# PeterChg/koordinator

Measured on AMD Instinct MI355X. Metric: pod×node Filter+Score evals/sec (LoadAwareScheduling + NodeResourcesFit, matrix mode), higher is better.
Workload: dtype int64

## Files before the change

### koordinator_amd/csrc/kg_engine.hip

```cpp
#include <dlfcn.h>
#include <hip/hip_runtime.h>
#include <rccl/rccl.h>
#include <stdarg.h>
#include <stdio.h>
#include <string.h>

#include <algorithm>
#include <map>
#include <unordered_map>
#include <utility>
#include <string>
#include <type_traits>
#include <vector>

#include "kg_comm.h"
#include "kg_common.h"
#include "kg_host.h"

#define KG_POD_CHUNK 64
#define KG_RESOLVE_THREADS 512
#define KG_RESOLVE_LA_T0 448
#define KG_CLS_ITEM_MAX 512
#define KG_MAX_CHUNK KG_PLACE_CHUNK_MAX
#define KG_MAX_TILES 4096
// ... 222 lines not shown
    if (POW2) return s >> shift;
    return (uint32_t)__builtin_fmaf((float)s, rcp, 0x1p-12f);
}

template <int S>
__device__ __forceinline__ kg_pod_hot_t<S> load_pod(const kg_pod_hot_t<S> *__restrict__ p) {
    constexpr int NB = sizeof(kg_pod_hot_t<S>) / 64;
    union U {
        kg_u32x16 v[NB];
        kg_pod_hot_t<S> h;
        __device__ U() {}
    } u;
    const kg_u32x16 *src = reinterpret_cast<const kg_u32x16 *>(p);
#pragma unroll
    for (int i = 0; i < NB; i++) u.v[i] = src[i];
    return u.h;
}

struct HotArgs {
    int32_t n_pods;
    int32_t pods_per_block;
    int32_t tile_begin;
    int32_t tiles_total;
    int64_t node_end;
    int64_t col_begin;
    int64_t score_stride;
    int32_t mask_words;
    uint32_t fit_cap;
    int32_t slot_res[8];
    int64_t now_ns;
    int32_t lax_n;
    int32_t lax_x[KG_LAX];
    uint32_t lax_w[KG_LAX];
    const double *lax_est;
};

template <int S, bool LA_PROD, bool LAX = false>
struct HotNode {
    int64_t fr[S];
    double R[S], F[S];
    double laR[2], laF0[2], laF1[2];
    double lxR[LAX ? KG_LAX : 1], lxF0[LAX ? KG_LAX : 1], lxF1[LAX ? KG_LAX : 1];
    uint32_t okbits;
    uint32_t slot_mask;
};

template <int S, bool LA_PROD, bool LAX = false>
__device__ __forceinline__ void load_hot_node(const kg_consts &c, const kg_planes &pl, const HotArgs &a, int64_t node,
                                              uint32_t slot_natives, HotNode<S, LA_PROD, LAX> &n) {
    const int64_t cap = pl.cap;
    const bool in_range = node < a.node_end;
    const uint32_t df = in_range ? pl.dflags[node] : 0u;
    const bool slow = (df & (LAX ? KGD_XSLOW : KGD_SLOW)) != 0;
    const uint32_t nfm = in_range ? pl.fit_mask[node] : 0u;
    n.slot_mask = 0;
#pragma unroll
    for (int s = 0; s < S; s++) {
        const int r = a.slot_res[s];
// ... 215 lines not shown
        __syncthreads();
        if (TOPK) {
            for (int pp = wave; pp < p1 - p0; pp += KG_BLOCK / 64) {
                const uint32_t t = tile_topk(kbuf + pp * 2 * KG_BLOCK);
                if (lane < KG_TOPK) partials[((int64_t)(p0 + pp) * a.tiles_total + tile) * KG_PARTIAL_SLOTS + lane] = t;
            }
            __syncthreads();
            continue;
        }
        const uint4 *src = reinterpret_cast<const uint4 *>(kbuf + rj * KG_BLOCK + rg * 16);
        uint32_t mx = 0;
#pragma unroll
        for (int k = 0; k < 4; k++) {
            const uint4 v = src[k];
            const uint32_t a0 = v.x > v.y ? v.x : v.y, a1 = v.z > v.w ? v.z : v.w;
            const uint32_t a2 = a0 > a1 ? a0 : a1;
            mx = mx > a2 ? mx : a2;
        }
        mx = dpp_max_step(mx, 0);
        mx = dpp_max_step(mx, 1);
        mx = dpp_max_step(mx, 2);
        mx = dpp_max_step(mx, 3);
        mx = dpp_max_step(mx, 4);
        if (rg == 31 && rj < p1 - p0) partials[(int64_t)(p0 + rj) * a.tiles_total + tile] = mx;
        __syncthreads();
    }
}

template <int NC, int NF>
struct ClsNode {
    int64_t fr[NC];
    double R[NF], F[NF];
    uint32_t w;
    uint32_t cq;
    bool ok;
    bool la_use;
};
struct ClsLa {
    double laR[2], laF[2];
};

template <int NC, int NF, bool MOST, bool FIT_ON, bool LA_ON>
__device__ __forceinline__ void load_cls_node(const kg_consts &c, const kg_planes &pl, const kg_cls_desc &d,
                                              int64_t node, int64_t node_end, int64_t now_ns, ClsNode<NC, NF> &n) {
    const int64_t cap = pl.cap;
    const bool in_range = node < node_end;
    const uint32_t df = in_range ? pl.dflags[node] : 0u;
// ... 308 lines not shown
                    __builtin_nontemporal_store(u32x4{v.x, v.y, v.z, v.w}, reinterpret_cast<u32x4 *>(scores + off + col0 + s8 * 8));
                }
            }
            if (lane < np && seg[0]) {
                uint64_t *mw = mask + (int64_t)cur[lane] * a.mask_words + (col0 >> 6);
                mw[0] = mb[0];
                if (seg[1]) mw[1] = mb[1];
            }
        }
        lds_barrier();
        if (wave == ci % (BT / 64)) {
            const int p = lane >> 3, q = lane & 7;
            const uint4 *src = reinterpret_cast<const uint4 *>(kcur + kg_kofs(p)) + q;
            uint32_t mx = 0;
#pragma unroll
            for (int k = 0; k < 16; k++) {
                const uint4 v = src[8 * k];
                mx = max(mx, max(max(v.x, v.y), max(v.z, v.w)));
            }
            mx = max(mx, (uint32_t)__builtin_amdgcn_update_dpp(0, (int)mx, 0x141, 0xf, 0xf, false));
            mx = max(mx, (uint32_t)__builtin_amdgcn_update_dpp(0, (int)mx, 0x4e, 0xf, 0xf, false));
            mx = max(mx, (uint32_t)__builtin_amdgcn_update_dpp(0, (int)mx, 0xb1, 0xf, 0xf, false));
            if (q == 0 && p < p1 - p0) {
                partials[(int64_t)cur[p] * a.tiles_total + tile] = mx;
            }
        }
    }
}

template <int NC, int NF, bool MOST, bool FIT_ON, bool LA_ON, bool OUT, bool W1>
__device__ __forceinline__ void cls_block_dup(const kg_consts &c, const kg_planes &pl, const HotArgs &a, const kg_cls_desc &d,
                                              const kg_cls_work &w, const char *__restrict__ rows_base,
                                              const int32_t *__restrict__ ids, uint64_t *__restrict__ mask,
                                              uint16_t *__restrict__ scores, uint32_t *__restrict__ partials,
                                              uint32_t *kbuf, int32_t *lid, uint16_t *lux, int32_t *cst, uint16_t *sstage,
                                              uint4 *mstage) {
    constexpr int CC = KG_EVAL3_CC;
    constexpr int BT = KG_TILE / 2;
    constexpr int SEGW = 128;
    static_assert(CC == 8 && BT == 512, "the key reduction maps one wave's lanes to 8 rows × 8 lanes");
    const int tid = threadIdx.x;
    const int lane = tid & 63;
    const int wave = __builtin_amdgcn_readfirstlane(tid >> 6);
    const int tile = a.tile_begin + w.tile;
    const int64_t wave_base = (int64_t)tile * KG_TILE + wave * SEGW;
    ClsNode<NC, NF> n[2];
    ClsLa la[2];
// ... 79 lines not shown
                        *reinterpret_cast<uint4 *>(mw) = v;
                    } else {
                        mw[0] = (uint64_t)v.x | ((uint64_t)v.y << 32);
                    }
                }
            }
        }
        if (wave == ci % (BT / 64)) {
            const int p = lane >> 3, q = lane & 7;
            const uint4 *src = reinterpret_cast<const uint4 *>(kcur + kg_kofs(p)) + q;
            uint32_t mx = 0;
#pragma unroll
            for (int k = 0; k < 16; k++) {
                const uint4 v = src[8 * k];
                mx = max(mx, max(max(v.x, v.y), max(v.z, v.w)));
            }
            mx = max(mx, (uint32_t)__builtin_amdgcn_update_dpp(0, (int)mx, 0x141, 0xf, 0xf, false));
            mx = max(mx, (uint32_t)__builtin_amdgcn_update_dpp(0, (int)mx, 0x4e, 0xf, 0xf, false));
            mx = max(mx, (uint32_t)__builtin_amdgcn_update_dpp(0, (int)mx, 0xb1, 0xf, 0xf, false));
            for (int m = m0; m < m1; m += 64) {
                const int mm = m + lane;
                const int u = mm < m1 ? lux[mm] - u0 : 0;
                const uint32_t k = (uint32_t)__builtin_amdgcn_ds_bpermute(u << 5, (int)mx);
                if (mm < m1) partials[(int64_t)lid[mm] * a.tiles_total + tile] = k;
            }
        }
    }
}

template <bool MOST, bool FIT_ON, bool LA_ON, bool OUT, bool W1, int KIND>
__global__ __launch_bounds__(KG_TILE / 2) __attribute__((amdgpu_waves_per_eu(KIND == 0 ? KG_EVAL3_WPE0 : KIND == 2 ? 5 : 4))) void k_eval3_dup(kg_consts c, kg_planes pl, HotArgs a,
                                                        const kg_cls_desc *__restrict__ descs,
                                                        const kg_cls_work *__restrict__ work, int32_t n_items,
                                                        const char *__restrict__ rows, const int32_t *__restrict__ ids,
                                                        uint64_t *__restrict__ mask, uint16_t *__restrict__ scores,
                                                        uint32_t *__restrict__ partials) {
    constexpr int CC = KG_EVAL3_CC, BT = KG_TILE / 2;
    __shared__ __attribute__((aligned(16))) uint32_t kbuf[2 * KG_KBUF_DW];
    static_assert(CC * BT <= 4096, "a chunk's keys fit the key buffer");
    __shared__ int32_t lid[KG_CLS_ITEM_MAX];
    __shared__ uint16_t lux[KG_CLS_ITEM_MAX];
    __shared__ int32_t cst[KG_CLS_ITEM_MAX / CC + 1];
    __shared__ __attribute__((aligned(16))) uint16_t sstage[OUT ? (BT / 64) * CC * 128 : 8];
    __shared__ uint4 mstage[2 * CC * 8];
    const int per = (int)(gridDim.x / KG_XCDS);
    const int item = (int)(blockIdx.x % KG_XCDS) * per + (int)(blockIdx.x / KG_XCDS);
    if (item >= n_items) return;
// ... 30 lines not shown
}

template <int VB>
__global__ __launch_bounds__(256) void k_eq_rows(const int32_t *__restrict__ of, int32_t P, const char *__restrict__ src,
                                                 char *__restrict__ dst, int64_t row_bytes) {
    typedef uint32_t vec_t __attribute__((ext_vector_type(VB / 4)));
    const int64_t nv = row_bytes / VB;
    for (int32_t p = blockIdx.y; p < P; p += gridDim.y) {
        const vec_t *s = reinterpret_cast<const vec_t *>(src + (int64_t)of[p] * row_bytes);
        vec_t *d = reinterpret_cast<vec_t *>(dst + (int64_t)p * row_bytes);
        for (int64_t i = (int64_t)blockIdx.x * blockDim.x + threadIdx.x; i < nv; i += (int64_t)gridDim.x * blockDim.x)
            __builtin_nontemporal_store(s[i], d + i);
    }
}

__global__ void k_slow_list(const uint32_t *__restrict__ dflags, int64_t begin, int64_t end, int32_t *__restrict__ list,
                            int32_t *__restrict__ count, uint32_t bit = KGD_SLOW) {
    const int64_t i = begin + (int64_t)blockIdx.x * blockDim.x + threadIdx.x;
    if (i < end && (dflags[i] & bit) && (dflags[i] & KGD_VALID)) list[atomicAdd(count, 1)] = (int32_t)i;
}

__global__ void k_fix_slow(kg_consts c, kg_planes pl, const kg_pod_dev *__restrict__ pods, int32_t n_pods,
                           const int32_t *__restrict__ list, const int32_t *__restrict__ count, int64_t col_begin,
                           int64_t col_end, int32_t mask_words, int64_t score_stride, int32_t tiles_total,
                           int64_t now_ns, unsigned long long *mask, uint16_t *scores, uint32_t *partials) {
    const int p = blockIdx.x * blockDim.x + threadIdx.x;
    if (p >= n_pods) return;
    const int32_t n = *count;
    for (int32_t k = 0; k < n; k++) {
        const int64_t node = list[k];
        if (node < col_begin || node >= col_end) continue;
        bool feas;
        uint32_t fit, la;
        kg_pair_exact(c, pl.rows[node], pl.dflags[node], pods[p], now_ns, feas, fit, la);
        const int64_t col = node - col_begin;
        if (scores) scores[(int64_t)p * score_stride + col] = (uint16_t)(fit | (la << 8));
        if (feas) {
            if (mask) atomicOr(&mask[(int64_t)p * mask_words + (col >> 6)], 1ull << (col & 63));
            const uint32_t tot = (uint32_t)c.weight_fit * fit + (uint32_t)c.weight_la * la;
            const uint32_t key = ((tot + 1u) << KG_TILE_SHIFT) | (uint32_t)(KG_TILE - 1 - (node % KG_TILE));
            atomicMax(&partials[(int64_t)p * tiles_total + node / KG_TILE], key);
        }
    }
}

__global__ __launch_bounds__(256) void k_eval_exact(kg_consts c, kg_planes pl, const kg_pod_dev *__restrict__ pods,
                                                    int32_t n_pods, int64_t begin, int64_t end, int32_t mask_words,
                                                    int64_t score_stride, int32_t tiles_total, int64_t now_ns,
                                                    unsigned long long *mask, uint16_t *scores, uint32_t *partials) {
    const int64_t col = (int64_t)blockIdx.x * 256 + threadIdx.x;
    const int64_t node = begin + col;
    const bool in = node < end;
    const uint32_t df = in ? pl.dflags[node] : 0u;
    const bool own = in && !(df & KGD_RSV);
    for (int p = blockIdx.y; p < n_pods; p += gridDim.y) {
        bool feas = false;
        uint32_t fit = 0, la = 0;
        if (own) kg_pair_exact(c, pl.rows[node], df, pods[p], now_ns, feas, fit, la);
        if (own && scores) scores[(int64_t)p * score_stride + col] = (uint16_t)(fit | (la << 8));
        const unsigned long long word = __builtin_amdgcn_ballot_w64(feas);
        if (mask && (threadIdx.x & 63) == 0 && (col >> 6) < mask_words && in) mask[(int64_t)p * mask_words + (col >> 6)] = word;
        uint32_t key = 0;
        if (feas) {
            const uint32_t tot = (uint32_t)c.weight_fit * fit + (uint32_t)c.weight_la * la;
            key = ((tot + 1u) << KG_TILE_SHIFT) | (uint32_t)(KG_TILE - 1 - (node % KG_TILE));
        }
        key = wave_max_u32(key);
        if ((threadIdx.x & 63) == 0 && key) atomicMax(&partials[(int64_t)p * tiles_total + node / KG_TILE], key);
    }
}

__global__ __launch_bounds__(256) void k_numa_bind_fix(kg_consts c, kg_planes pl, HotArgs a, const kg_pod_dev *__restrict__ pods,
                                                       unsigned long long *mask, uint16_t *scores, uint8_t *numa_scores,
                                                       uint32_t *partials) {
    const int64_t col = (int64_t)blockIdx.x * 256 + threadIdx.x;
    const int64_t node = a.col_begin + col;
    if (node >= a.node_end) return;
    const kg_node_row &row = pl.rows[node];
    if (!(row.flags & KG_NODE_NUMA_OPTIONS) || row.numa_policy == KG_NUMA_NONE || row.n_zones <= 0 ||
        !(row.flags & KG_NODE_NUMA_TOPO_VALID))
        return;
    const BatchMasks bm{0xFFu, 0xFFu};
    for (int p = blockIdx.y; p < a.n_pods; p += gridDim.y) {
        const kg_pod_dev &pd = pods[p];
        if (pd.flags & (KG_POD_NUMA_SKIP | KG_POD_NUMA_BIND_INVALID)) continue;
        const bool bind = (pd.flags & KG_POD_NUMA_CPU_BIND) ||
                          (row.node_cpu_bind != KG_NODE_CPU_BIND_NONE && pd.numa_req[KG_RES_CPU] != 0);
        if (!bind) continue;
        NodeRegs n;
        load_node(c, pl, node, true, bm, a.now_ns, n);
        uint32_t fit = 0, la = 0;
        bool ok = eval_pair(c, pl, pd, n, node, a.now_ns, fit, la);
        kg_numa_out o;
        kg_numa_pair_z<kg_zone_calc, true>(c, row, pd, o, kg_zone_calc{row});
        ok = ok && o.feasible;
        if (scores) scores[(int64_t)p * a.score_stride + col] = (uint16_t)(fit | (la << 8));
        if (numa_scores) numa_scores[(int64_t)p * a.score_stride + col] = (uint8_t)o.score;
        if (ok) {
            if (mask) atomicOr(&mask[(int64_t)p * a.mask_words + (col >> 6)], 1ull << (col & 63));
            const uint32_t key = ((total_of(c, fit, la, o.score) + 1u) << KG_TILE_SHIFT) | (uint32_t)(KG_TILE - 1 - (node % KG_TILE));
            atomicMax(&partials[(int64_t)p * a.tiles_total + node / KG_TILE], key);
        }
    }
}

#define KG_NUMA2_NODES 256
#define KG_NUMA2_SEG 32
#define KG_NUMA2_SEG_TOPK 8
#ifndef KG_NUMA2_WPE
#define KG_NUMA2_WPE 3
#endif
typedef uint32_t kg_u32x4 __attribute__((ext_vector_type(4)));
#ifndef KG_NUMA2_FLUSH
#define KG_NUMA2_FLUSH 32
#endif
#ifndef KG_NUMA2_PREFETCH
#define KG_NUMA2_PREFETCH 1
#endif
__device__ __forceinline__ void kg_glds16(const uint4 *src, uint4 *slot) {
    const uint32_t lds = __builtin_amdgcn_readfirstlane((uint32_t)(uintptr_t)slot);
    int keep;
    asm volatile("s_mov_b32 %0, m0\n\ts_mov_b32 m0, %2\n\ts_nop 0\n\tglobal_load_lds_dwordx4 %1, off\n\ts_mov_b32 m0, %0"
                 : "=&s"(keep) : "v"(src), "s"(lds) : "memory");
}
// ... 162 lines not shown
            }
            if (live && numa_scores && c0 < a.score_stride) {
                kg_u32x4 *d = reinterpret_cast<kg_u32x4 *>(numa_scores + (int64_t)p * a.score_stride + c0);
#pragma unroll
                for (int i = 0; i < FL / 16; i++)
                    __builtin_nontemporal_store(kg_u32x4{nacc[4 * i], nacc[4 * i + 1], nacc[4 * i + 2], nacc[4 * i + 3]}, d + i);
            }
#pragma unroll
            for (int i = 0; i < FL / 2; i++) sacc[i] = 0u;
#pragma unroll
            for (int i = 0; i < FL / 4; i++) nacc[i] = 0u;
        }
        if ((k & 63) == 63) {
            const int64_t c0 = col - 63;
            if (live && mask && c0 < (int64_t)a.mask_words * 64) mask[(int64_t)p * a.mask_words + (c0 >> 6)] = mword;
            mword = 0;
        }
    }
    if (npw & 63) {
        const int64_t c0 = base + npw - 32 - a.col_begin;
        if (live && mask && c0 < (int64_t)a.mask_words * 64)
            reinterpret_cast<uint32_t *>(mask + (int64_t)p * a.mask_words)[c0 >> 5] = (uint32_t)mword;
    }
    if (live && best) atomicMax(&partials[(int64_t)p * a.tiles_total + tile], best);
}

template <bool COMBINE>
__global__ __launch_bounds__(256) __attribute__((amdgpu_waves_per_eu(KG_NUMA2_WPE))) void k_eval_numa2(kg_consts c, kg_planes pl, HotArgs a,
                                                    const kg_pod_dev *__restrict__ pods,
                                                    const kg_node_row *__restrict__ rows,
                                                    unsigned long long *__restrict__ mask,
                                                    uint16_t *__restrict__ scores, uint8_t *__restrict__ numa_scores,
                                                    uint32_t *__restrict__ partials, const int32_t *__restrict__ perm,
                                                    BatchMasks bm, int32_t *queue, int32_t n_items, int32_t seg) {
    const int tid = threadIdx.x, lane = tid & 63;
    const int wave = __builtin_amdgcn_readfirstlane(tid >> 6);
    __shared__ kg_zone_tab_data ztab[256 / 64];
    __shared__ __attribute__((aligned(16))) uint4 lrow_s[256 / 64][KG_NUMA2_PREFETCH ? 2 : 1][64];
    static_assert(sizeof(kg_node_row) % 16 == 0 && sizeof(kg_node_row) <= 64 * 16, "rows are staged as 16-byte words");
    const int n_pb = (a.n_pods + 63) / 64;
    for (int it = 0;; it++) {
        int64_t tile, base;
        int npw, pb;
        if (queue == nullptr) {
            if (it > 0) break;
            tile = (int64_t)a.tile_begin + blockIdx.x;
            pb = blockIdx.y;
// ... 5 lines not shown
            item = __builtin_amdgcn_readfirstlane(item);
            if (item >= n_items) break;
            pb = item % n_pb;
            const int run = item / n_pb;
            tile = (int64_t)a.tile_begin + run / (KG_TILE / seg);
            base = (int64_t)a.tile_begin * KG_TILE + (int64_t)run * seg;
            npw = seg;
        }
        const int slot = pb * 64 + lane;
        const bool live = slot < a.n_pods;
        const int p = live && perm ? perm[slot] : slot;
        const kg_pod_dev pd = pods[live ? p : 0];
        numa2_run<COMBINE>(c, pl, a, pd, p, live, tile, base, npw, rows, mask, scores, numa_scores, partials, bm, ztab[wave],
                  &lrow_s[wave][0][0]);
    }
}

__device__ __forceinline__ unsigned long long decode_partial(uint32_t k, int tile) {
    if (k == 0) return 0ull;
    const uint32_t node = (uint32_t)tile * KG_TILE + (KG_TILE - 1) - (k & (KG_TILE - 1));
    return ((unsigned long long)(k >> KG_TILE_SHIFT) << 32) | (0xFFFFFFFFull - node);
}

__global__ void k_top1(const uint32_t *__restrict__ partials, int32_t tiles, int32_t n_pods,
                       unsigned long long *__restrict__ out) {
    const int wave = (blockIdx.x * blockDim.x + threadIdx.x) >> 6;
    const int lane = threadIdx.x & 63;
    if (wave >= n_pods) return;
    unsigned long long best = 0;
    for (int t = lane; t < tiles; t += 64) {
        unsigned long long k = decode_partial(partials[(int64_t)wave * tiles + t], t);
        best = best > k ? best : k;
    }
    best = wave_max_u64(best);
    if (lane == 0) out[wave] = best;
}

template <bool NUMA>
__device__ unsigned long long pair_key(const kg_consts &c, const kg_planes &pl, const kg_pod_dev &p, int64_t node,
                                       int64_t n_nodes, int64_t now_ns) {
    if (node < 0 || node >= n_nodes) return 0ull;
    NodeRegs n;
    BatchMasks bm{0xFFu, 0xFFu};
    load_node(c, pl, node, true, bm, now_ns, n);
    uint32_t fit, la, numa = 0;
    if (!eval_pair(c, pl, p, n, node, now_ns, fit, la)) return 0ull;
    if (NUMA && (c.plugins & KG_PLUGIN_NUMA)) {
        const uint64_t ns = kg_numa_eval_any(c, pl.rows[node], p);
        if (!(ns >> 32)) return 0ull;
        numa = (uint32_t)ns;
    }
    return ((unsigned long long)(total_of(c, fit, la, numa) + 1u) << 32) | (0xFFFFFFFFull - (unsigned long long)node);
}

#define KG_NUMA_CHUNK_PODS 16
#define KG_CHUNK_WPE 3
template <bool BZ>
__global__ __launch_bounds__(256) __attribute__((amdgpu_waves_per_eu(KG_CHUNK_WPE))) void k_eval_numa_chunk(kg_consts c, kg_planes pl, HotArgs a,
// ... 1693 lines not shown
            hipLaunchKernelGGL((k_eval3_dup<MOST, FIT_ON, LA_ON, true, W1, KIND>), g1, dim3(KG_TILE / 2), 0, stream,
                               e->consts, e->pl, a, descs, work + first, count, rows, ids, mask, scores, partials);
        else
            hipLaunchKernelGGL((k_eval3_dup<MOST, FIT_ON, LA_ON, false, W1, KIND>), g1, dim3(KG_TILE / 2), 0, stream,
                               e->consts, e->pl, a, descs, work + first, count, rows, ids, mask, scores, partials);
    } else {
        grid.y = (unsigned)count;
        if (mask)
            hipLaunchKernelGGL((k_eval3<MOST, FIT_ON, LA_ON, true, W1, KIND, LAU>), grid, dim3(KG_TILE / 2), 0, stream,
                               e->consts, e->pl, a, descs, work + first, rows, ids, mask, scores, partials);
        else
            hipLaunchKernelGGL((k_eval3<MOST, FIT_ON, LA_ON, false, W1, KIND, LAU>), grid, dim3(KG_TILE / 2), 0, stream,
                               e->consts, e->pl, a, descs, work + first, rows, ids, mask, scores, partials);
    }
}

template <bool MOST, bool FIT_ON, bool LA_ON, bool W1>
void launch_cls4(kg_engine *e, dim3 grid, const HotArgs &a, uint64_t *mask, uint16_t *scores, uint32_t *partials) {
    const char *m = (const char *)e->cls_mem;
    const kg_cls_desc *descs = (const kg_cls_desc *)m;
    const kg_cls_work *work = (const kg_cls_work *)(m + e->cls_work_off);
    const char *rows = m + e->cls_rows_off;
    const int32_t *ids = (const int32_t *)(m + e->cls_ids_off);
    if (!e->stream2) {
        (void)hipStreamCreateWithFlags(&e->stream2, hipStreamNonBlocking);
        (void)hipEventCreateWithFlags(&e->ev_fork, hipEventDisableTiming);
        (void)hipEventCreateWithFlags(&e->ev_join, hipEventDisableTiming);
    }
    (void)hipEventRecord(e->ev_fork, e->stream);
    (void)hipStreamWaitEvent(e->stream2, e->ev_fork, 0);
    hipStream_t s2 = e->stream2;
#define KG_LAUNCH_KIND(K)                                                                                              \
    launch_cls_kind<MOST, FIT_ON, LA_ON, W1, K, 2>(e, grid, a, descs, work, rows, ids, mask, scores, partials, e->stream); \
    launch_cls_kind<MOST, FIT_ON, LA_ON, W1, K, 1>(e, grid, a, descs, work, rows, ids, mask, scores, partials, e->stream); \
    launch_cls_kind<MOST, FIT_ON, LA_ON, W1, K, 0>(e, grid, a, descs, work, rows, ids, mask, scores, partials, s2)
    KG_LAUNCH_KIND(0);
    KG_LAUNCH_KIND(1);
    KG_LAUNCH_KIND(2);
    KG_LAUNCH_KIND(3);
#undef KG_LAUNCH_KIND
    (void)hipEventRecord(e->ev_join, s2);
    (void)hipStreamWaitEvent(e->stream, e->ev_join, 0);
}

template <bool MOST, bool FIT_ON, bool LA_ON>
void launch_cls3(kg_engine *e, dim3 grid, const HotArgs &a, uint64_t *mask, uint16_t *scores, uint32_t *partials) {
    bool unit = e->consts.weight_fit == 1 && e->consts.weight_la == 1;
    if (LA_ON) unit = unit && e->consts.la_w[0] == 1 && e->consts.la_w[1] == 1;
    for (const kg_cls_desc &d : e->cls_desc)
        for (int f = 0; f < 4; f++) unit = unit && d.fit_w[f] <= 1u && d.uni_w[f] <= 1u;
    if (unit) launch_cls4<MOST, FIT_ON, LA_ON, true>(e, grid, a, mask, scores, partials);
    else launch_cls4<MOST, FIT_ON, LA_ON, false>(e, grid, a, mask, scores, partials);
}

void launch_cls(kg_engine *e, dim3 grid, const HotArgs &a, uint64_t *mask, uint16_t *scores, uint32_t *partials) {
    const bool most = e->consts.fit_most != 0;
    const bool fit = (e->consts.plugins & KG_PLUGIN_FIT) != 0, la = (e->consts.plugins & KG_PLUGIN_LOADAWARE) != 0;
    if (!fit) launch_cls3<false, false, true>(e, grid, a, mask, scores, partials);
    else if (most && la) launch_cls3<true, true, true>(e, grid, a, mask, scores, partials);
    else if (most) launch_cls3<true, true, false>(e, grid, a, mask, scores, partials);
    else if (la) launch_cls3<false, true, true>(e, grid, a, mask, scores, partials);
    else launch_cls3<false, true, false>(e, grid, a, mask, scores, partials);
}

kg_status slow_refresh(kg_engine *e) {
    if (e->slow_valid) return KG_OK;
    HIP_TRY(e, hipMemsetAsync(e->slow_count, 0, sizeof(int32_t), e->stream));
    if (e->n_nodes > 0)
        hipLaunchKernelGGL(k_slow_list, dim3((unsigned)((e->n_nodes + 255) / 256)), dim3(256), 0, e->stream, e->pl.dflags,
                           (int64_t)0, e->n_nodes, e->slow_list, e->slow_count);
    HIP_TRY(e, hipGetLastError());
    e->slow_valid = true;
    return KG_OK;
}

kg_status launch_eval_plain(kg_engine *e, int64_t now_ns, int32_t pod_begin, int32_t n, uint64_t *mask, uint16_t *scores,
                            uint32_t *partials, bool use_cls, bool topk, HotArgs a, int64_t shard_tiles, bool prof = true) {
    if (e->consts.la_extra && !topk && e->lax_ok) {
        a.lax_n = e->lax_n;
        for (int k = 0; k < KG_LAX; k++) {
            a.lax_x[k] = k < e->lax_n ? e->lax_x[k] : 0;
            a.lax_w[k] = k < e->lax_n ? (uint32_t)e->consts.la_wx[e->lax_x[k]] : 0u;
        }
        a.lax_est = e->hot_lax + (int64_t)pod_begin * KG_LAX;
        if (prof && e->profiling) HIP_TRY(e, prof_begin(e));
        dim3 grid((unsigned)shard_tiles, (unsigned)((n + a.pods_per_block - 1) / a.pods_per_block));
        const bool prod = e->la_prod;
#define KG_LAX_LAUNCH(S_)                                                                                               \
        do {                                                                                                            \
            const kg_pod_hot_t<S_> *hp = reinterpret_cast<const kg_pod_hot_t<S_> *>(e->hot) + pod_begin;                \
            if (mask && prod)                                                                                          \
                hipLaunchKernelGGL((k_eval2<S_, false, true, true, false, true>), grid, dim3(KG_BLOCK), 0, e->stream,  \
                                   e->consts, e->pl, a, hp, mask, scores, partials);                                   \
            else if (mask)                                                                                             \
                hipLaunchKernelGGL((k_eval2<S_, false, false, true, false, true>), grid, dim3(KG_BLOCK), 0, e->stream, \
                                   e->consts, e->pl, a, hp, mask, scores, partials);                                   \
            else if (prod)                                                                                             \
                hipLaunchKernelGGL((k_eval2<S_, false, true, false, false, true>), grid, dim3(KG_BLOCK), 0, e->stream, \
                                   e->consts, e->pl, a, hp, mask, scores, partials);                                   \
            else                                                                                                       \
                hipLaunchKernelGGL((k_eval2<S_, false, false, false, false, true>), grid, dim3(KG_BLOCK), 0, e->stream,\
                                   e->consts, e->pl, a, hp, mask, scores, partials);                                   \
        } while (0)
        if (e->nslot == 2) KG_LAX_LAUNCH(2);
        else if (e->nslot == 4) KG_LAX_LAUNCH(4);
        else KG_LAX_LAUNCH(8);
#undef KG_LAX_LAUNCH
        HIP_TRY(e, hipGetLastError());
        if (prof && e->profiling) HIP_TRY(e, prof_end(e));
        HIP_TRY(e, hipMemsetAsync(e->xslow_count, 0, sizeof(int32_t), e->stream));
        if (e->n_nodes > 0)
            hipLaunchKernelGGL(k_slow_list, dim3((unsigned)((e->n_nodes + 255) / 256)), dim3(256), 0, e->stream, e->pl.dflags,
                               (int64_t)0, e->n_nodes, e->xslow_list, e->xslow_count, (uint32_t)KGD_XSLOW);
        hipLaunchKernelGGL(k_fix_slow, dim3((unsigned)((n + 255) / 256)), dim3(256), 0, e->stream, e->consts, e->pl,
                           e->pods + pod_begin, n, e->xslow_list, e->xslow_count, e->shard_begin, e->shard_end,
                           a.mask_words, a.score_stride, a.tiles_total, now_ns, (unsigned long long *)mask, scores,
                           partials);
        HIP_TRY(e, hipGetLastError());
        return KG_OK;
    }
    if (e->consts.la_extra && !topk) {
        if (prof && e->profiling) HIP_TRY(e, prof_begin(e));
        const int64_t width = e->shard_end - e->shard_begin;
        dim3 grid((unsigned)((width + 255) / 256), (unsigned)(n < 65535 ? n : 65535));
        hipLaunchKernelGGL(k_eval_exact, grid, dim3(256), 0, e->stream, e->consts, e->pl, e->pods + pod_begin, n,
                           e->shard_begin, e->shard_end, a.mask_words, a.score_stride, a.tiles_total, now_ns,
                           (unsigned long long *)mask, scores, partials);
        HIP_TRY(e, hipGetLastError());
        if (prof && e->profiling) HIP_TRY(e, prof_end(e));
        return KG_OK;
    }
    use_cls = use_cls && e->cls_ok && !e->reps_in && pod_begin == 0 && n == e->n_pods;
    if (use_cls) {
        kg_status st = cls_layout(e, e->shard_end - e->shard_begin, shard_tiles);
        if (st) return st;
    }
    dim3 grid((unsigned)shard_tiles, use_cls ? (unsigned)e->cls_nwork : (unsigned)((n + a.pods_per_block - 1) / a.pods_per_block));
    if (prof && e->profiling) HIP_TRY(e, prof_begin(e));
    if (use_cls) launch_cls(e, grid, a, mask, scores, partials);
    else if (e->nslot == 2) launch_hot<2>(e, grid, a, pod_begin, mask, scores, partials, topk);
    else if (e->nslot == 4) launch_hot<4>(e, grid, a, pod_begin, mask, scores, partials, topk);
    else launch_hot<8>(e, grid, a, pod_begin, mask, scores, partials, topk);
    HIP_TRY(e, hipGetLastError());
    if (prof && e->profiling) HIP_TRY(e, prof_end(e));
    kg_status st = slow_refresh(e);
    if (st) return st;
    if (!topk) {
        hipLaunchKernelGGL(k_fix_slow, dim3((unsigned)((n + 255) / 256)), dim3(256), 0, e->stream, e->consts, e->pl,
                           e->pods + pod_begin, n, e->slow_list, e->slow_count, e->shard_begin, e->shard_end,
                           a.mask_words, a.score_stride, a.tiles_total, now_ns, (unsigned long long *)mask, scores,
                           partials);
        HIP_TRY(e, hipGetLastError());
    }
    return KG_OK;
}

kg_status launch_eval(kg_engine *e, int64_t now_ns, int32_t pod_begin, int32_t n, uint64_t *mask, uint16_t *scores,
                      uint32_t *partials, bool use_cls = false, uint8_t *numa_scores = nullptr, bool topk = false) {
    if (n <= 0) return KG_OK;
    if ((mask == nullptr) != (scores == nullptr)) return set_err(e, KG_ERR_INVALID_ARG, "mask and scores go together");
    const int64_t shard_tiles = (e->shard_end - e->shard_begin + KG_TILE - 1) / KG_TILE;
    if (shard_tiles <= 0) return KG_OK;
    HotArgs a;
    a.n_pods = n;
    a.pods_per_block = pods_per_block_for(n, shard_tiles);
    a.tile_begin = (int32_t)(e->shard_begin / KG_TILE);
    a.tiles_total = (int32_t)tiles_total(e);
    a.node_end = e->shard_end;
    a.col_begin = e->shard_begin;
    a.mask_words = (int32_t)((e->shard_end - e->shard_begin + 63) / 64);
    a.score_stride = (e->shard_end - e->shard_begin + 63) / 64 * 64;
    a.fit_cap = e->consts.fit_most ? 100u : 0xFFFFFFFFu;
    for (int s = 0; s < 8; s++) a.slot_res[s] = s < e->nslot ? e->slot_res[s] : -1;
    a.now_ns = now_ns;
    if ((e->consts.plugins & KG_PLUGIN_NUMA) && topk && n <= e->numa_chunk_pods) {
        if (e->profiling) HIP_TRY(e, prof_begin(e));
        const unsigned blocks = (unsigned)((shard_tiles + KG_XCDS - 1) / KG_XCDS * KG_XCDS * n);
        if (e->ncache_live && !e->consts.numa_bz)
            hipLaunchKernelGGL(k_eval_numa_cached, dim3(blocks), dim3(256), 0, e->stream, e->consts, e->pl, a,
                               e->pods + pod_begin, (int32_t)shard_tiles, partials, e->ncache, e->eq_of + pod_begin,
                               e->ncache_stride, e->eq_n);
        else if (e->consts.numa_bz)
            hipLaunchKernelGGL(k_eval_numa_chunk<true>, dim3(blocks), dim3(256), 0, e->stream, e->consts, e->pl, a,
                               e->pods + pod_begin, (int32_t)shard_tiles, partials);
        else
            hipLaunchKernelGGL(k_eval_numa_chunk<false>, dim3(blocks), dim3(256), 0, e->stream, e->consts, e->pl, a,
                               e->pods + pod_begin, (int32_t)shard_tiles, partials);
        HIP_TRY(e, hipGetLastError());
        if (e->profiling) HIP_TRY(e, prof_end(e));
        return KG_OK;
// ... 41 lines not shown
                while (z < KG_NUMA2_NODES / 32 && blocks * z < 2 * e->numa_resident_wgs) z *= 2;
                dim3 grid((unsigned)shard_tiles, (unsigned)((n + 63) / 64), z);
                if (combine)
                    hipLaunchKernelGGL(k_eval_numa2<true>, grid, dim3(256), 0, e->stream, e->consts, e->pl, a, e->pods + pod_begin,
                                       e->pl.rows, (unsigned long long *)mask, scores, numa_scores, partials, perm, bm,
                                       (int32_t *)nullptr, 0, 0);
                else
                    hipLaunchKernelGGL(k_eval_numa2<false>, grid, dim3(256), 0, e->stream, e->consts, e->pl, a, e->pods + pod_begin,
                                       e->pl.rows, (unsigned long long *)mask, scores, numa_scores, partials, perm, bm,
                                       (int32_t *)nullptr, 0, 0);
            }
        }
        HIP_TRY(e, hipGetLastError());
        if ((!topk || e->consts.numa_bz) && e->n_numa_policy_nodes > 0 && (e->batch_bind || e->n_node_bind_nodes > 0)) {
            const int64_t width = e->shard_end - e->shard_begin;
            dim3 grid((unsigned)((width + 255) / 256), (unsigned)(n < 65535 ? n : 65535));
            hipLaunchKernelGGL(k_numa_bind_fix, grid, dim3(256), 0, e->stream, e->consts, e->pl, a, e->pods + pod_begin,
                               (unsigned long long *)mask, scores, numa_scores, partials);
            HIP_TRY(e, hipGetLastError());
        }
        if (e->profiling) HIP_TRY(e, prof_end(e));
        return KG_OK;
    }
    return launch_eval_plain(e, now_ns, pod_begin, n, mask, scores, partials, use_cls, topk, a, shard_tiles);
}

#define KG_RSV_POD_CHUNK 1024

RsvArgs rsv_args(const kg_engine *e) {
    RsvArgs ra{};
    if ((e->consts.plugins & KG_PLUGIN_RESERVATION) && e->n_rn > 0) {
        ra.rsv = e->rsv;
        ra.rfirst = e->rfirst;
        ra.rnode = e->rnode;
        ra.n_rn = e->n_rn;
        ra.E = e->rsv_e;
        ra.O = e->rsv_o;
        const int32_t ng = (e->n_rn + KG_RSV_GROUP - 1) / KG_RSV_GROUP;
        if (ng <= KG_RSV_MAX_GROUPS) {
            ra.M = e->rsv_m;
            ra.Mn = e->rsv_mn;
            ra.G = e->rsv_g;
            ra.ngroups = ng;
        }
    }
    if (e->consts.plugins & KG_PLUGIN_ELASTICQUOTA) ra.quota = e->quota;
    ra.quota_parent = e->cfg.eq_check_parent_quota != 0;
// ... 548 lines not shown
        else scores = (uint16_t *)out->scores;
    }
    uint8_t *numa = nullptr;
    if (out->numa_scores) {
        if (stage_numa) { numa = (uint8_t *)q; q += up(numa_b); }
        else numa = out->numa_scores;
        if (!numa_on && numa_b) HIP_TRY(e, hipMemsetAsync(numa, 0, numa_b, e->stream));
    }
    uint8_t *rsvp = nullptr;
    if (out->rsv_scores) {
        if (stage_rsv) { rsvp = (uint8_t *)q; q += up(numa_b); }
        else rsvp = out->rsv_scores;
        if (numa_b) HIP_TRY(e, hipMemsetAsync(rsvp, 0, numa_b, e->stream));
    }
    const RsvArgs ra = rsv_args(e);
    st = quota_ready(e);
    if (st) return st;
    const bool gated = (ra.quota || ra.rsv) && P > 0;
    if (gated) {
        hipLaunchKernelGGL(k_pod_gate, dim3((unsigned)((P + 255) / 256)), dim3(256), 0, e->stream, ra.quota, ra.quota_parent, e->pods, P,
                           e->gate);
        HIP_TRY(e, hipGetLastError());
    }
    HIP_TRY(e, hipMemsetAsync(part, 0, part_b, e->stream));
    st = launch_eval(e, now_ns, 0, P, mask, scores, part, true, numa_on ? numa : nullptr);
    if (st) return st;
    unsigned long long *tdst = out->top1 ? (dev ? (unsigned long long *)out->top1 : top) : nullptr;
    if (tdst && P > 0) {
        hipLaunchKernelGGL(k_top1, dim3((unsigned)((P + 3) / 4)), dim3(256), 0, e->stream, part, (int32_t)T, P, tdst);
        HIP_TRY(e, hipGetLastError());
    }
    const int32_t mask_words = (int32_t)((width + 63) / 64);
    const int64_t stride = (width + 63) / 64 * 64;
    if (gated) {
        hipLaunchKernelGGL(k_quota_apply, dim3((unsigned)P), dim3(256), 0, e->stream, e->gate + P, P,
                           (unsigned long long *)mask, mask_words, tdst, (uint8_t *)nullptr, stride);
        HIP_TRY(e, hipGetLastError());
    }
    if (ra.rsv) {
        for (int32_t b = 0; b < P; b += KG_RSV_POD_CHUNK) {
            const int32_t n = P - b < KG_RSV_POD_CHUNK ? P - b : KG_RSV_POD_CHUNK;
            st = rsv_eval_chunk(e, now_ns, b, n, mask ? mask + (int64_t)b * mask_words : nullptr,
                                scores ? scores + (int64_t)b * stride : nullptr,
                                numa_on && numa ? numa + (int64_t)b * stride : nullptr, mask_words, stride);
            if (st) return st;
            hipLaunchKernelGGL(k_rsv_reduce, dim3((unsigned)n), dim3(256), 0, e->stream, e->consts, ra, n,
                               tdst ? tdst + b : nullptr, rsvp ? rsvp + (int64_t)b * stride : nullptr, e->shard_begin,
                               e->shard_end, stride);
            HIP_TRY(e, hipGetLastError());
        }
    }
    if (ra.quota && P > 0) {
        hipLaunchKernelGGL(k_quota_apply, dim3((unsigned)P), dim3(256), 0, e->stream, e->gate, P,
                           (unsigned long long *)mask, mask_words, tdst, rsvp, stride);
        HIP_TRY(e, hipGetLastError());
    }
    if (!dev) {
        if (out->top1 && P > 0) HIP_TRY(e, hipMemcpyAsync(out->top1, top, top_b, hipMemcpyDeviceToHost, e->stream));
        if (out->mask && P > 0) HIP_TRY(e, hipMemcpyAsync(out->mask, mask, mask_b, hipMemcpyDeviceToHost, e->stream));
        if (out->scores && P > 0) HIP_TRY(e, hipMemcpyAsync(out->scores, scores, score_b, hipMemcpyDeviceToHost, e->stream));
        if (out->numa_scores && P > 0) HIP_TRY(e, hipMemcpyAsync(out->numa_scores, numa, numa_b, hipMemcpyDeviceToHost, e->stream));
        if (out->rsv_scores && P > 0) HIP_TRY(e, hipMemcpyAsync(out->rsv_scores, rsvp, numa_b, hipMemcpyDeviceToHost, e->stream));
        HIP_TRY(e, hipStreamSynchronize(e->stream));
    }
    return KG_OK;
}

}

namespace {

kg_status eval_eq(kg_engine *e, int64_t now_ns, const kg_eval_out *out) {
    const int32_t P = e->n_pods, U = e->eq_n;
    const int64_t width = e->shard_end - e->shard_begin;
    const int64_t words = (width + 63) / 64, stride = words * 64;
    const size_t rb[5] = {(size_t)words * 8, (size_t)stride * 2, 8, (size_t)stride, (size_t)stride};
    void *const want[5] = {out->mask, out->scores, out->top1, out->numa_scores, out->rsv_scores};
    const bool dev = out->out_on_device != 0;
    auto up = [](size_t b) { return (b + 255) / 256 * 256; };
    size_t need = 0, off_c[5] = {}, off_s[5] = {};
    for (int k = 0; k < 5; k++)
        if (want[k]) { off_c[k] = need; need += up(rb[k] * (size_t)U); }
    for (int k = 0; k < 5; k++)
        if (want[k] && !dev) { off_s[k] = need; need += up(rb[k] * (size_t)P); }
    if (need > e->eq_mem_bytes) {
        HIP_TRY(e, hipStreamSynchronize(e->stream));
        if (e->eq_mem) HIP_TRY(e, hipFree(e->eq_mem));
        e->eq_mem = nullptr;
// ... 1032 lines not shown
```

Measured before the change: 2373 billion.

## Store partial keys tile-major, fuse slow-node fixup into parallel top1 reduction

Adds configurable pod/tile strides so matrix-mode partials are written tile-major, letting a new top1 kernel read coalesced across 64 pods with 16 tile slices per block. In the non-atomic path it drops the partials memset and folds the slow-node exact fixup into the top1 kernel rather than launching k_fix_slow. It also skips the secondary-stream fork/join when no class work needs it. The aim is to cut launches, memsets and strided top1 reads, at the cost of relying on every tile key being written by the eval kernels and on added bounds checks.

Result: faster. 2510 billion, median of 6 (+5.8%).

```diff
diff --git a/koordinator_amd/csrc/kg_engine.hip b/koordinator_amd/csrc/kg_engine.hip
--- a/koordinator_amd/csrc/kg_engine.hip
+++ b/koordinator_amd/csrc/kg_engine.hip
@@ -268,6 +268,7 @@
     int32_t pods_per_block;
     int32_t tile_begin;
     int32_t tiles_total;
+    int32_t key_pod, key_tile;
     int64_t node_end;
     int64_t col_begin;
     int64_t score_stride;
@@ -280,6 +281,10 @@
     uint32_t lax_w[KG_LAX];
     const double *lax_est;
 };
+
+__device__ __forceinline__ int64_t kg_key_index(int64_t pod, int64_t tile, int32_t key_pod, int32_t key_tile) {
+    return pod * key_pod + tile * key_tile;
+}
 
 template <int S, bool LA_PROD, bool LAX = false>
 struct HotNode {
@@ -541,7 +546,7 @@
         mx = dpp_max_step(mx, 2);
         mx = dpp_max_step(mx, 3);
         mx = dpp_max_step(mx, 4);
-        if (rg == 31 && rj < p1 - p0) partials[(int64_t)(p0 + rj) * a.tiles_total + tile] = mx;
+        if (rg == 31 && rj < p1 - p0) partials[kg_key_index(p0 + rj, tile, a.key_pod, a.key_tile)] = mx;
         __syncthreads();
     }
 }
@@ -896,7 +901,7 @@
             mx = max(mx, (uint32_t)__builtin_amdgcn_update_dpp(0, (int)mx, 0x4e, 0xf, 0xf, false));
             mx = max(mx, (uint32_t)__builtin_amdgcn_update_dpp(0, (int)mx, 0xb1, 0xf, 0xf, false));
             if (q == 0 && p < p1 - p0) {
-                partials[(int64_t)cur[p] * a.tiles_total + tile] = mx;
+                partials[kg_key_index(cur[p], tile, a.key_pod, a.key_tile)] = mx;
             }
         }
     }
@@ -1022,7 +1027,7 @@
                 const int mm = m + lane;
                 const int u = mm < m1 ? lux[mm] - u0 : 0;
                 const uint32_t k = (uint32_t)__builtin_amdgcn_ds_bpermute(u << 5, (int)mx);
-                if (mm < m1) partials[(int64_t)lid[mm] * a.tiles_total + tile] = k;
+                if (mm < m1) partials[kg_key_index(lid[mm], tile, a.key_pod, a.key_tile)] = k;
             }
         }
     }
@@ -1099,7 +1104,7 @@
 
 __global__ void k_fix_slow(kg_consts c, kg_planes pl, const kg_pod_dev *__restrict__ pods, int32_t n_pods,
                            const int32_t *__restrict__ list, const int32_t *__restrict__ count, int64_t col_begin,
-                           int64_t col_end, int32_t mask_words, int64_t score_stride, int32_t tiles_total,
+                           int64_t col_end, int32_t mask_words, int64_t score_stride, int32_t key_pod, int32_t key_tile,
                            int64_t now_ns, unsigned long long *mask, uint16_t *scores, uint32_t *partials) {
     const int p = blockIdx.x * blockDim.x + threadIdx.x;
     if (p >= n_pods) return;
@@ -1116,14 +1121,14 @@
             if (mask) atomicOr(&mask[(int64_t)p * mask_words + (col >> 6)], 1ull << (col & 63));
             const uint32_t tot = (uint32_t)c.weight_fit * fit + (uint32_t)c.weight_la * la;
             const uint32_t key = ((tot + 1u) << KG_TILE_SHIFT) | (uint32_t)(KG_TILE - 1 - (node % KG_TILE));
-            atomicMax(&partials[(int64_t)p * tiles_total + node / KG_TILE], key);
+            atomicMax(&partials[kg_key_index(p, node / KG_TILE, key_pod, key_tile)], key);
         }
     }
 }
 
 __global__ __launch_bounds__(256) void k_eval_exact(kg_consts c, kg_planes pl, const kg_pod_dev *__restrict__ pods,
                                                     int32_t n_pods, int64_t begin, int64_t end, int32_t mask_words,
-                                                    int64_t score_stride, int32_t tiles_total, int64_t now_ns,
+                                                    int64_t score_stride, int32_t key_pod, int32_t key_tile, int64_t now_ns,
                                                     unsigned long long *mask, uint16_t *scores, uint32_t *partials) {
     const int64_t col = (int64_t)blockIdx.x * 256 + threadIdx.x;
     const int64_t node = begin + col;
@@ -1143,7 +1148,7 @@
             key = ((tot + 1u) << KG_TILE_SHIFT) | (uint32_t)(KG_TILE - 1 - (node % KG_TILE));
         }
         key = wave_max_u32(key);
-        if ((threadIdx.x & 63) == 0 && key) atomicMax(&partials[(int64_t)p * tiles_total + node / KG_TILE], key);
+        if ((threadIdx.x & 63) == 0 && key) atomicMax(&partials[kg_key_index(p, node / KG_TILE, key_pod, key_tile)], key);
     }
 }
 
@@ -1176,7 +1181,7 @@
         if (ok) {
             if (mask) atomicOr(&mask[(int64_t)p * a.mask_words + (col >> 6)], 1ull << (col & 63));
             const uint32_t key = ((total_of(c, fit, la, o.score) + 1u) << KG_TILE_SHIFT) | (uint32_t)(KG_TILE - 1 - (node % KG_TILE));
-            atomicMax(&partials[(int64_t)p * a.tiles_total + node / KG_TILE], key);
+            atomicMax(&partials[kg_key_index(p, node / KG_TILE, a.key_pod, a.key_tile)], key);
         }
     }
 }
@@ -1385,7 +1390,7 @@
         if (live && mask && c0 < (int64_t)a.mask_words * 64)
             reinterpret_cast<uint32_t *>(mask + (int64_t)p * a.mask_words)[c0 >> 5] = (uint32_t)mword;
     }
-    if (live && best) atomicMax(&partials[(int64_t)p * a.tiles_total + tile], best);
+    if (live && best) atomicMax(&partials[kg_key_index(p, tile, a.key_pod, a.key_tile)], best);
 }
 
 template <bool COMBINE>
@@ -1437,18 +1442,53 @@
     return ((unsigned long long)(k >> KG_TILE_SHIFT) << 32) | (0xFFFFFFFFull - node);
 }
 
-__global__ void k_top1(const uint32_t *__restrict__ partials, int32_t tiles, int32_t n_pods,
-                       unsigned long long *__restrict__ out) {
-    const int wave = (blockIdx.x * blockDim.x + threadIdx.x) >> 6;
-    const int lane = threadIdx.x & 63;
-    if (wave >= n_pods) return;
+#define KG_TOP1_PODS 64
+#define KG_TOP1_SLICES 16
+template <bool FIX>
+__global__ __launch_bounds__(KG_TOP1_PODS * KG_TOP1_SLICES) void k_top1(
+    const uint32_t *__restrict__ partials, int32_t n_pods, int32_t tile_begin, int32_t shard_tiles, int32_t tiles_total,
+    unsigned long long *__restrict__ out, kg_consts c, kg_planes pl, const kg_pod_dev *__restrict__ pods,
+    const int32_t *__restrict__ list, const int32_t *__restrict__ count, int64_t col_begin, int64_t col_end,
+    int32_t mask_words, int64_t score_stride, int64_t now_ns, unsigned long long *mask, uint16_t *scores) {
+    __shared__ unsigned long long sbest[KG_TOP1_SLICES - 1][KG_TOP1_PODS];
+    const int lane = threadIdx.x & (KG_TOP1_PODS - 1);
+    const int slice = threadIdx.x / KG_TOP1_PODS;
+    const int p = blockIdx.x * KG_TOP1_PODS + lane;
+    const bool live = p < n_pods;
     unsigned long long best = 0;
-    for (int t = lane; t < tiles; t += 64) {
-        unsigned long long k = decode_partial(partials[(int64_t)wave * tiles + t], t);
-        best = best > k ? best : k;
-    }
-    best = wave_max_u64(best);
-    if (lane == 0) out[wave] = best;
+    if (live) {
+#pragma unroll 8
+        for (int t = tile_begin + slice; t < tile_begin + shard_tiles; t += KG_TOP1_SLICES) {
+            const int64_t i = kg_key_index(p, t, 1, n_pods);
+            if (!KG_IN(60, i, (int64_t)tiles_total * n_pods)) continue;
+            const unsigned long long k = decode_partial(partials[i], t);
+            best = best > k ? best : k;
+        }
+    }
+    if (slice > 0) sbest[slice - 1][lane] = best;
+    __syncthreads();
+    if (slice > 0 || !live) return;
+#pragma unroll
+    for (int s = 0; s < KG_TOP1_SLICES - 1; s++) best = best > sbest[s][lane] ? best : sbest[s][lane];
+    if (FIX) {
+        const int32_t n = *count;
+        for (int32_t k = 0; k < n; k++) {
+            const int64_t node = list[k];
+            if (node < col_begin || node >= col_end) continue;
+            bool feas;
+            uint32_t fit, la;
+            kg_pair_exact(c, pl.rows[node], pl.dflags[node], pods[p], now_ns, feas, fit, la);
+            const int64_t col = node - col_begin;
+            if (scores && KG_IN(61, col, score_stride)) scores[(int64_t)p * score_stride + col] = (uint16_t)(fit | (la << 8));
+            if (feas) {
+                if (mask && KG_IN(62, col >> 6, mask_words)) atomicOr(&mask[(int64_t)p * mask_words + (col >> 6)], 1ull << (col & 63));
+                const uint32_t tot = (uint32_t)c.weight_fit * fit + (uint32_t)c.weight_la * la;
+                const unsigned long long key = ((unsigned long long)(tot + 1u) << 32) | (0xFFFFFFFFull - (unsigned long long)node);
+                best = best > key ? best : key;
+            }
+        }
+    }
+    out[p] = best;
 }
 
 template <bool NUMA>
@@ -3188,14 +3228,18 @@
     const kg_cls_work *work = (const kg_cls_work *)(m + e->cls_work_off);
     const char *rows = m + e->cls_rows_off;
     const int32_t *ids = (const int32_t *)(m + e->cls_ids_off);
-    if (!e->stream2) {
-        (void)hipStreamCreateWithFlags(&e->stream2, hipStreamNonBlocking);
-        (void)hipEventCreateWithFlags(&e->ev_fork, hipEventDisableTiming);
-        (void)hipEventCreateWithFlags(&e->ev_join, hipEventDisableTiming);
-    }
-    (void)hipEventRecord(e->ev_fork, e->stream);
-    (void)hipStreamWaitEvent(e->stream2, e->ev_fork, 0);
-    hipStream_t s2 = e->stream2;
+    bool fork = false;
+    for (int k = 0; k < 4; k++) fork = fork || e->cls_kind_work[3 * k + 0][1] > 0;
+    if (fork) {
+        if (!e->stream2) {
+            (void)hipStreamCreateWithFlags(&e->stream2, hipStreamNonBlocking);
+            (void)hipEventCreateWithFlags(&e->ev_fork, hipEventDisableTiming);
+            (void)hipEventCreateWithFlags(&e->ev_join, hipEventDisableTiming);
+        }
+        (void)hipEventRecord(e->ev_fork, e->stream);
+        (void)hipStreamWaitEvent(e->stream2, e->ev_fork, 0);
+    }
+    hipStream_t s2 = fork ? e->stream2 : e->stream;
 #define KG_LAUNCH_KIND(K)                                                                                              \
     launch_cls_kind<MOST, FIT_ON, LA_ON, W1, K, 2>(e, grid, a, descs, work, rows, ids, mask, scores, partials, e->stream); \
     launch_cls_kind<MOST, FIT_ON, LA_ON, W1, K, 1>(e, grid, a, descs, work, rows, ids, mask, scores, partials, e->stream); \
@@ -3205,8 +3249,10 @@
     KG_LAUNCH_KIND(2);
     KG_LAUNCH_KIND(3);
 #undef KG_LAUNCH_KIND
-    (void)hipEventRecord(e->ev_join, s2);
-    (void)hipStreamWaitEvent(e->stream, e->ev_join, 0);
+    if (fork) {
+        (void)hipEventRecord(e->ev_join, s2);
+        (void)hipStreamWaitEvent(e->stream, e->ev_join, 0);
+    }
 }
 
 template <bool MOST, bool FIT_ON, bool LA_ON>
@@ -3241,7 +3287,9 @@
 }
 
 kg_status launch_eval_plain(kg_engine *e, int64_t now_ns, int32_t pod_begin, int32_t n, uint64_t *mask, uint16_t *scores,
-                            uint32_t *partials, bool use_cls, bool topk, HotArgs a, int64_t shard_tiles, bool prof = true) {
+                            uint32_t *partials, bool use_cls, bool topk, HotArgs a, int64_t shard_tiles, bool prof = true,
+                            bool *defer_slow = nullptr) {
+    if (defer_slow) *defer_slow = false;
     if (e->consts.la_extra && !topk && e->lax_ok) {
         a.lax_n = e->lax_n;
         for (int k = 0; k < KG_LAX; k++) {
@@ -3280,7 +3328,7 @@
                                (int64_t)0, e->n_nodes, e->xslow_list, e->xslow_count, (uint32_t)KGD_XSLOW);
         hipLaunchKernelGGL(k_fix_slow, dim3((unsigned)((n + 255) / 256)), dim3(256), 0, e->stream, e->consts, e->pl,
                            e->pods + pod_begin, n, e->xslow_list, e->xslow_count, e->shard_begin, e->shard_end,
-                           a.mask_words, a.score_stride, a.tiles_total, now_ns, (unsigned long long *)mask, scores,
+                           a.mask_words, a.score_stride, a.key_pod, a.key_tile, now_ns, (unsigned long long *)mask, scores,
                            partials);
         HIP_TRY(e, hipGetLastError());
         return KG_OK;
@@ -3290,7 +3338,7 @@
         const int64_t width = e->shard_end - e->shard_begin;
         dim3 grid((unsigned)((width + 255) / 256), (unsigned)(n < 65535 ? n : 65535));
         hipLaunchKernelGGL(k_eval_exact, grid, dim3(256), 0, e->stream, e->consts, e->pl, e->pods + pod_begin, n,
-                           e->shard_begin, e->shard_end, a.mask_words, a.score_stride, a.tiles_total, now_ns,
+                           e->shard_begin, e->shard_end, a.mask_words, a.score_stride, a.key_pod, a.key_tile, now_ns,
                            (unsigned long long *)mask, scores, partials);
         HIP_TRY(e, hipGetLastError());
         if (prof && e->profiling) HIP_TRY(e, prof_end(e));
@@ -3311,10 +3359,12 @@
     if (prof && e->profiling) HIP_TRY(e, prof_end(e));
     kg_status st = slow_refresh(e);
     if (st) return st;
-    if (!topk) {
+    if (!topk && defer_slow) {
+        *defer_slow = true;
+    } else if (!topk) {
         hipLaunchKernelGGL(k_fix_slow, dim3((unsigned)((n + 255) / 256)), dim3(256), 0, e->stream, e->consts, e->pl,
                            e->pods + pod_begin, n, e->slow_list, e->slow_count, e->shard_begin, e->shard_end,
-                           a.mask_words, a.score_stride, a.tiles_total, now_ns, (unsigned long long *)mask, scores,
+                           a.mask_words, a.score_stride, a.key_pod, a.key_tile, now_ns, (unsigned long long *)mask, scores,
                            partials);
         HIP_TRY(e, hipGetLastError());
     }
@@ -3322,7 +3372,10 @@
 }
 
 kg_status launch_eval(kg_engine *e, int64_t now_ns, int32_t pod_begin, int32_t n, uint64_t *mask, uint16_t *scores,
-                      uint32_t *partials, bool use_cls = false, uint8_t *numa_scores = nullptr, bool topk = false) {
+                      uint32_t *partials, bool use_cls = false, uint8_t *numa_scores = nullptr, bool topk = false,
+                      bool tile_major = false, bool *defer_slow = nullptr) {
+    if (defer_slow) *defer_slow = false;
+    if (tile_major && topk) return set_err(e, KG_ERR_INVALID_ARG, "placement partials are pod-major");
     if (n <= 0) return KG_OK;
     if ((mask == nullptr) != (scores == nullptr)) return set_err(e, KG_ERR_INVALID_ARG, "mask and scores go together");
     const int64_t shard_tiles = (e->shard_end - e->shard_begin + KG_TILE - 1) / KG_TILE;
@@ -3332,6 +3385,8 @@
     a.pods_per_block = pods_per_block_for(n, shard_tiles);
     a.tile_begin = (int32_t)(e->shard_begin / KG_TILE);
     a.tiles_total = (int32_t)tiles_total(e);
+    a.key_pod = tile_major ? 1 : a.tiles_total;
+    a.key_tile = tile_major ? n : 1;
     a.node_end = e->shard_end;
     a.col_begin = e->shard_begin;
     a.mask_words = (int32_t)((e->shard_end - e->shard_begin + 63) / 64);
@@ -3419,7 +3474,7 @@
         if (e->profiling) HIP_TRY(e, prof_end(e));
         return KG_OK;
     }
-    return launch_eval_plain(e, now_ns, pod_begin, n, mask, scores, partials, use_cls, topk, a, shard_tiles);
+    return launch_eval_plain(e, now_ns, pod_begin, n, mask, scores, partials, use_cls, topk, a, shard_tiles, true, defer_slow);
 }
 
 #define KG_RSV_POD_CHUNK 1024
@@ -4014,12 +4069,23 @@
                            e->gate);
         HIP_TRY(e, hipGetLastError());
     }
-    HIP_TRY(e, hipMemsetAsync(part, 0, part_b, e->stream));
-    st = launch_eval(e, now_ns, 0, P, mask, scores, part, true, numa_on ? numa : nullptr);
+    unsigned long long *tdst = out->top1 ? (dev ? (unsigned long long *)out->top1 : top) : nullptr;
+    const bool atomic_keys = numa_on || e->consts.la_extra;
+    if (atomic_keys) HIP_TRY(e, hipMemsetAsync(part, 0, part_b, e->stream));
+    bool slow_owed = false;
+    st = launch_eval(e, now_ns, 0, P, mask, scores, part, true, numa_on ? numa : nullptr, false, true,
+                     !atomic_keys && tdst ? &slow_owed : nullptr);
     if (st) return st;
-    unsigned long long *tdst = out->top1 ? (dev ? (unsigned long long *)out->top1 : top) : nullptr;
     if (tdst && P > 0) {
-        hipLaunchKernelGGL(k_top1, dim3((unsigned)((P + 3) / 4)), dim3(256), 0, e->stream, part, (int32_t)T, P, tdst);
+        const int64_t shard_tiles = width > 0 ? (width + KG_TILE - 1) / KG_TILE : 0;
+        const dim3 grid((unsigned)((P + KG_TOP1_PODS - 1) / KG_TOP1_PODS)), block(KG_TOP1_PODS * KG_TOP1_SLICES);
+#define KG_TOP1_ARGS                                                                                                   \
+    part, P, (int32_t)(e->shard_begin / KG_TILE), (int32_t)shard_tiles, (int32_t)T, tdst, e->consts, e->pl, e->pods,   \
+        e->slow_list, e->slow_count, e->shard_begin, e->shard_end, (int32_t)((width + 63) / 64),                       \
+        (int64_t)((width + 63) / 64 * 64), now_ns, (unsigned long long *)mask, scores
+        if (slow_owed) hipLaunchKernelGGL(k_top1<true>, grid, block, 0, e->stream, KG_TOP1_ARGS);
+        else hipLaunchKernelGGL(k_top1<false>, grid, block, 0, e->stream, KG_TOP1_ARGS);
+#undef KG_TOP1_ARGS
         HIP_TRY(e, hipGetLastError());
     }
     const int32_t mask_words = (int32_t)((width + 63) / 64);
@@ -4055,7 +4121,7 @@
         if (out->rsv_scores && P > 0) HIP_TRY(e, hipMemcpyAsync(out->rsv_scores, rsvp, numa_b, hipMemcpyDeviceToHost, e->stream));
         HIP_TRY(e, hipStreamSynchronize(e->stream));
     }
-    return KG_OK;
+    return bounds_verdict(e);
 }
 
 }
```
